# Picsart-AI-Research/MI-GAN

Hardware: AMD Instinct MI355X
Metric: images/sec migan-512 generator fwd (higher is better)
Workload: dtype f32; 1 GPU; migan-512 generator forward, batch=32 per GPU, 512x512, fp32 (BASELINE configs[2]); global_batch=32, resolution=512, parallelism=batch-shard x1, activation_storage=f32, streams=2, weights=static (migan_assume_static_weights: 1x1 operand planes prepared once)

## Files before the change

### mi-gan_amd/csrc/migan_pipe.hpp

```cpp
#pragma once

namespace migan {

constexpr int kPipeBWaves = 8;
constexpr int pipe_threads(int na) { return (na + kPipeBWaves) * 64; }

template <int MODE, int NT, int CIN, bool FROMRGB, int R>
struct PipeLds {
  static constexpr int NKC = CIN / 32;
  static constexpr int IN_SLOT = 1536 * 16;
  static constexpr int A_BUF = 2 * 128 * 64;
  static constexpr int B_CHUNK = 2 * NT * 64;
  static constexpr bool WRES = NKC * B_CHUNK <= 32 * 1024;
  static constexpr int NBUF_B = WRES ? NKC : 2;
  static constexpr int OFF_IN = 0;
  static constexpr int OFF_A = OFF_IN + R * IN_SLOT;
  static constexpr int OFF_B = OFF_A + 2 * A_BUF;
  static constexpr int OFF_W = OFF_B + NBUF_B * B_CHUNK;
  static constexpr bool TAPS_RES = NKC <= 8;
  static constexpr int OFF_F = OFF_W + (TAPS_RES ? NKC : 2) * 1280;
  static constexpr int F_SZ = FROMRGB ? NKC * 3 * 32 * 32 : 0;
  static constexpr int OFF_RGB = OFF_F + F_SZ;
  static constexpr int RGB_BUF = 192 * 32;
  static constexpr int OFF_T = OFF_RGB + (FROMRGB ? 2 * RGB_BUF : 0);
// ... 532 lines not shown

  if constexpr (MODE == MODE_NORMAL) {
    float* const t_s = reinterpret_cast<float*>(lds + L::OFF_T) + wb * (32 * 32);
    const int q4 = lane & 7, prow = lane >> 3;
    int twr[4];
    {
      const int u = (l31 >> 2) ^ (2 * half);
#pragma unroll
      for (int v = 0; v < 4; ++v) twr[v] = (4 * half) * 32 + ((u ^ ((v & 1) + 4 * (v >> 1))) << 2) + (l31 & 3);
    }
    const int trd0 = prow * 32 + ((q4 ^ (prow >> 1)) << 2), trd1 = prow * 32 + ((q4 ^ (prow >> 1) ^ 4) << 2);
    float nz[4] = {0.f, 0.f, 0.f, 0.f};
    float nzn[4] = {0.f, 0.f, 0.f, 0.f};
    float rs[4][3];
    unsigned pix0 = 0;
    f4 tw[NTIW][3];
    float tbias[3] = {0.f, 0.f, 0.f};
    if constexpr (TORGB) {
#pragma unroll
      for (int ch = 0; ch < 3; ++ch) tbias[ch] = p.trgb_b[ch];
#pragma unroll
      for (int j = 0; j < NTIW; ++j)
#pragma unroll
        for (int ch = 0; ch < 3; ++ch) tw[j][ch] = ld4(p.trgb_w + ch * p.CO + cbk * (NT / 2) + j * 32 + q4 * 4);
    }
    float* const part_s = reinterpret_cast<float*>(lds + L::OFF_P) + rb * (32 * 4);
    u4v u8c = {0u, 0u, 0u, 0u}, u8n = {0u, 0u, 0u, 0u};
    auto request_next = [&]() {
      if (has_noise) {
        const unsigned px = (unsigned)((cgy0 + 2 * rb) * p.WO + cgx0 + prow) * 4u;
#pragma unroll
        for (int q = 0; q < 4; ++q) nzn[q] = *at_bytes(p.noise + ((q >> 1) * p.WO + (q & 1) * 8), px);
      }
      if constexpr (TORGB) {
        if (p.u8_out && cbk == 0 && q4 < 4)
          u8n = fetch_pixel_bytes(p.u8_img, p.u8_mask, (size_t)cb0 * p.HO * p.WO + (size_t)(cgy0 + 2 * rb + (q4 >> 1)) * p.WO + cgx0 + (q4 & 1) * 8 + prow);
      }
    };
    auto begin_tile_epilogue = [&]() {
      pix0 = (unsigned)((pgy0 + 2 * rb) * p.WO + pgx0 + prow);
#pragma unroll
      for (int q = 0; q < 4; ++q) nz[q] = nzn[q];
      if constexpr (TORGB) {
        u8c = u8n;
#pragma unroll
        for (int q = 0; q < 4; ++q) rs[q][0] = rs[q][1] = rs[q][2] = 0.0f;
      }
    };
    auto stage_block = [&](const f16v& a) {
      MIGAN_WAVE_SYNC();
#pragma unroll
      for (int r = 0; r < 16; ++r) t_s[twr[((r >> 1) & 1) + 2 * ((r >> 2) & 1)] + ((r & 3) + 8 * (r >> 2)) * 32] = a[r];
      MIGAN_WAVE_SYNC();
    };
    f4 tv[4];
    auto fetch_block = [&]() {
#pragma unroll
      for (int q = 0; q < 4; ++q) tv[q] = ld4(t_s + ((q & 1) ? trd1 : trd0) + q * 8 * 32);
    };
    auto finish_block = [&](int j) {
      char* yb = reinterpret_cast<char*>(p.y) + (size_t)pb0 * img_out_bytes;
#pragma unroll
      for (int q = 0; q < 4; ++q) {
        f4 v = tv[q] * acc_scale + MIGAN_FMUL_RN(nz[q], ns);
        v = act4(v);
        const unsigned pix = pix0 + (unsigned)((q >> 1) * p.WO + (q & 1) * 8);
        Io<0>::st(yb, (pix * (unsigned)p.CO + (unsigned)(pn0 + cbk * (NT / 2) + j * 32 + q4 * 4)) * 4u, v);
        if constexpr (TORGB) {
          float r0, r1, r2;
          torgb_partial(v, tw[j][0], tw[j][1], tw[j][2], r0, r1, r2);
          rs[q][0] += r0; rs[q][1] += r1; rs[q][2] += r2;
        }
      }
    };
    float mine[3] = {0.f, 0.f, 0.f};
    auto rgb_partials = [&]() {
#pragma unroll
      for (int q = 0; q < 4; ++q) {
        const float s0 = MIGAN_SUM8(rs[q][0]), s1 = MIGAN_SUM8(rs[q][1]), s2 = MIGAN_SUM8(rs[q][2]);
        if (q4 == q) { mine[0] = s0; mine[1] = s1; mine[2] = s2; }
      }
      if (cbk == 1 && q4 < 4) st4(part_s + (8 * q4 + prow) * 4, f4{mine[0], mine[1], mine[2], 0.0f});
    };
    auto rgb_finish = [&]() {
      if (cbk == 0 && q4 < 4) {
        const f4 other = ld4(part_s + (8 * q4 + prow) * 4);
        const size_t plane = (size_t)p.HO * p.WO;
        const int oy = pgy0 + 2 * rb + (q4 >> 1), ox = pgx0 + (q4 & 1) * 8 + prow;
        float o3[3] = {mine[0] + other.x, mine[1] + other.y, mine[2] + other.z};
        MIGAN_OPAQUE_F(o3[0]); MIGAN_OPAQUE_F(o3[1]); MIGAN_OPAQUE_F(o3[2]);
        o3[0] += tbias[0]; MIGAN_OPAQUE_F(o3[0]);
        o3[1] += tbias[1]; MIGAN_OPAQUE_F(o3[1]);
        o3[2] += tbias[2]; MIGAN_OPAQUE_F(o3[2]);
        if (p.img_prev) {
          const int y0 = (oy & 1) ? (oy >> 1) : (oy >> 1) - 1, x0 = (ox & 1) ? (ox >> 1) : (ox >> 1) - 1;
          const float wy0 = (oy & 1) ? 0.75f : 0.25f, wx0 = (ox & 1) ? 0.75f : 0.25f;
          const float* pw = reinterpret_cast<const float*>(lds + L::OFF_PW + ppar * L::PW_SZ) + (y0 - (pgy0 >> 1) + 1) * 10 + (x0 - (pgx0 >> 1) + 1);
#pragma unroll
          for (int ch = 0; ch < 3; ++ch) {
            const float r0 = wx0 * pw[ch * 64] + (1.0f - wx0) * pw[ch * 64 + 1];
            const float r1 = wx0 * pw[ch * 64 + 10] + (1.0f - wx0) * pw[ch * 64 + 11];
            o3[ch] = (wy0 * r0 + (1.0f - wy0) * r1) + o3[ch];
          }
        }
        if (p.u8_out) {
          compose_pixel_bytes(u8c, p.u8_out, (size_t)pb0 * plane + (size_t)oy * p.WO + ox, o3[0], o3[1], o3[2]);
        } else {
          const unsigned po = (unsigned)(oy * p.WO + ox) * 4u;
#pragma unroll
          for (int ch = 0; ch < 3; ++ch) *at_bytes(p.img_out + ((size_t)pb0 * 3 + ch) * plane, po) = o3[ch];
        }
      }
    };
#pragma unroll
    for (int c = 0; c < NKC; ++c) {
      mfma_chunk(c & 1, WRES ? c : (c & 1), c == 0);
      if (c == NKC - 1) {
        request_next();
        stage_block(acc[0]);
        hand_over();
      }
      if constexpr (FROMRGB) build_step(bcur);
      MIGAN_BARRIER_LDS();
    }
    for (int t = 1; t < T; ++t) {
#pragma unroll
      for (int c = 0; c < NKC; ++c) {
        PPROF_MARK(7);
        if (c < NTIW) fetch_block();
        mfma_chunk(c & 1, WRES ? c : (c & 1), c == 0);
        PPROF_MARK(4);
        if (c == NKC - 1) request_next();
        PPROF_MARK(12);
        if (c == 0) begin_tile_epilogue();
        PPROF_MARK(5);
        if (c < NTIW) {
          finish_block(c);
          if (c + 1 < NTIW) stage_block(accp[c + 1 < NTIW ? c + 1 : 0]);
        }
        PPROF_MARK(9);
        if constexpr (TORGB) {
          if (c == NTIW - 1) rgb_partials();
          PPROF_MARK(10);
          if (c == NTIW) rgb_finish();
          PPROF_MARK(11);
        }
        if (c == NKC - 1) {
          stage_block(acc[0]);
          hand_over();
        }
        PPROF_MARK(7);
        if constexpr (FROMRGB) build_step(bcur);
        PPROF_MARK(13);
        MIGAN_BARRIER_LDS();
        PPROF_MARK(6);
      }
    }
    begin_tile_epilogue();
#pragma unroll
    for (int j = 0; j < NTIW; ++j) {
      fetch_block();
      finish_block(j);
      if (j + 1 < NTIW) stage_block(accp[j + 1 < NTIW ? j + 1 : 0]);
    }
    if constexpr (TORGB) {
      rgb_partials();
      MIGAN_BARRIER_LDS();
      rgb_finish();
    }
  } else {
    constexpr int GS = 64 + 4, QN = 16, LG_QN = 4, NH = NT / 64;
    static_assert(NT == 64 || NT == 128, "FIR-up tiles: 64 or 128 output channels");
    constexpr int SP = NKC / NH;
    static_assert(NKC % NH == 0 && SP >= 2, "too few K steps to hide the FIR epilogue under");
    constexpr int BT = kPipeBWaves * 64;
    constexpr int STEP = BT >> LG_QN;
    constexpr int ITEMS = MT * QN / BT;
    float* const g_s = reinterpret_cast<float*>(lds + L::OFF_T);
    auto acc_to_lds = [&](int h) {
      if (NH == 2 && cbk != h) return;
#pragma unroll
      for (int j = 0; j < NTIW; ++j)
#pragma unroll
        for (int r = 0; r < 16; ++r) {
          const int row = rb * 32 + (r & 3) + 8 * (r >> 2) + 4 * half;
          const int ly = pgy0 + (row >> lgGW), lx = pgx0 + (row & (GW - 1));
          float v = accp[j][r];
          if (ly < 0 || ly >= p.H || lx < 0 || lx >= p.W) v = 0.0f;
          g_s[row * GS + (NH == 2 ? j * 32 : cbk * 32) + l31] = v;
        }
    };
    const int c4 = tb & (QN - 1), m0 = tb >> LG_QN;
    struct ItemIo {
      f4 sk[2][2];
      float nzv[2][2];
    };
    auto item_geo = [&](int k, int h, int& m, unsigned& lpix, unsigned& loff) -> bool {
      m = m0 + k * STEP;
      const int gy = m >> lgGW, gx = m & (GW - 1);
      if (gy < 1 || gy > GH - 2 || gx < 1 || gx > GW - 2) return false;
      const int ly = pgy0 + gy, lx = pgx0 + gx;
      if (ly >= p.H || lx >= p.W) return false;
      lpix = (unsigned)((2 * ly) * p.WO + 2 * lx);
      loff = (lpix * (unsigned)p.CO + (unsigned)(pn0 + h * 64 + c4 * 4)) * 4u;
      return true;
    };
    auto item_load = [&](int k, int h, ItemIo& io) {
      int m;
      unsigned lpix, loff;
      if (!item_geo(k, h, m, lpix, loff)) return;
      const char* sb = p.skip ? reinterpret_cast<const char*>(p.skip) + (size_t)pb0 * img_out_bytes : nullptr;
#pragma unroll
      for (int a = 0; a < 2; ++a)
#pragma unroll
        for (int bb = 0; bb < 2; ++bb) {
          const unsigned dp = (unsigned)(a * p.WO + bb);
          io.nzv[a][bb] = has_noise ? p.noise[lpix + dp] : 0.0f;
          io.sk[a][bb] = sb ? Io<0>::ld_once(sb, loff + dp * (unsigned)p.CO * 4u) : f4{0.f, 0.f, 0.f, 0.f};
        }
    };
    auto item_finish = [&](int k, int h, const ItemIo& io) {
      int m;
      unsigned lpix, loff;
      if (!item_geo(k, h, m, lpix, loff)) return;
      char* yb = reinterpret_cast<char*>(p.y) + (size_t)pb0 * img_out_bytes;
      f4 e[3], o[3];
#pragma unroll
      for (int dy = 0; dy < 3; ++dy) {
        const float* gp = g_s + (m + (dy - 1) * GW) * GS + c4 * 4;
        const f4 l = ld4(gp - GS), ctr = ld4(gp), rgt = ld4(gp + GS);
        e[dy] = 0.25f * l + 0.75f * ctr;
        o[dy] = 0.75f * ctr + 0.25f * rgt;
      }
      f4 out[2][2];
      out[0][0] = 0.25f * e[0] + 0.75f * e[1];
      out[0][1] = 0.25f * o[0] + 0.75f * o[1];
      out[1][0] = 0.75f * e[1] + 0.25f * e[2];
      out[1][1] = 0.75f * o[1] + 0.25f * o[2];
#pragma unroll
      for (int a = 0; a < 2; ++a)
#pragma unroll
        for (int bb = 0; bb < 2; ++bb) {
          f4 v = out[a][bb] * acc_scale + MIGAN_FMUL_RN(io.nzv[a][bb], ns);
          v = act4(v);
          v += io.sk[a][bb];
          Io<0>::st(yb, loff + (unsigned)(a * p.WO + bb) * (unsigned)p.CO * 4u, v);
        }
    };
    constexpr int SL = SP - 1;
    auto slice_of = [](int k) { return k * SL / ITEMS; };
    ItemIo io[2];
#pragma unroll
    for (int c = 0; c < NKC; ++c) {
      mfma_chunk(c & 1, WRES ? c : (c & 1), c == 0);
      if (c == NKC - 1) hand_over();
      MIGAN_BARRIER_LDS();
    }
    for (int t = 1; t < T; ++t) {
#pragma unroll
      for (int c = 0; c < NKC; ++c) {
        constexpr int dummy = 0; (void)dummy;
        const int h = c / SP, cs = c % SP;
        if (cs >= 1) {
#pragma unroll
          for (int k = 0; k < ITEMS; ++k)
            if (slice_of(k) == cs - 1 && (k == 0 || slice_of(k - 1) != cs - 1)) item_load(k, h, io[k & 1]);
        }
        PPROF_MARK(7);
        mfma_chunk(c & 1, WRES ? c : (c & 1), c == 0);
        PPROF_MARK(4);
        if (cs == 0) {
          acc_to_lds(h);
        } else {
#pragma unroll
          for (int k = 0; k < ITEMS; ++k)
            if (slice_of(k) == cs - 1) {
              if (k + 1 < ITEMS && slice_of(k + 1) == cs - 1) item_load(k + 1, h, io[(k + 1) & 1]);
              item_finish(k, h, io[k & 1]);
            }
        }
        if (c == NKC - 1) hand_over();
        PPROF_MARK(5);
        MIGAN_BARRIER_LDS();
        PPROF_MARK(6);
      }
    }
#pragma unroll
    for (int h = 0; h < NH; ++h) {
      if (h > 0) MIGAN_BARRIER_LDS();
      acc_to_lds(h);
      MIGAN_BARRIER_LDS();
      item_load(0, h, io[0]);
#pragma unroll
      for (int k = 0; k < ITEMS; ++k) {
        if (k + 1 < ITEMS) item_load(k + 1, h, io[(k + 1) & 1]);
        item_finish(k, h, io[k & 1]);
      }
    }
  }
  PPROF_MARK(5);
  PPROF_END(AT);
}

template <int NT, int CIN, int R>
struct DownLds {
  static constexpr int KC = 16, NKC = CIN / KC;
  static constexpr int IN_UNITS = 12 * 36 * 4;
  static constexpr int A_BUF = 2 * 64 * 32;
  static constexpr int B_CHUNK = 2 * NT * 32;
  static constexpr bool WRES = NKC * B_CHUNK <= 32 * 1024;
  static constexpr int NBUF_B = WRES ? NKC : 2;
  static constexpr int DWP = 17;
  static constexpr int D_SZ = 10 * 2 * DWP * KC * 4;
  static constexpr int IN_SLOT = IN_UNITS * 16;
  static constexpr int OFF_D = R * IN_SLOT;
  static constexpr int OFF_A = OFF_D + D_SZ;
  static constexpr int OFF_B = OFF_A + 2 * A_BUF;
  static constexpr int OFF_W = OFF_B + NBUF_B * B_CHUNK;
  static constexpr int OFF_T = OFF_W + NKC * 640;
  template <int NB> static constexpr int total() { return OFF_T + NB * 32 * 32 * 4; }
};

template <int NT, int CIN, int R, int NA, int NB>
MIGAN_GLOBAL void MIGAN_LAUNCH_BOUNDS((NA + NB) * 64, (NA + NB) / 4) sepconv_pipedown_kernel(const SepArgs p) {
  typedef DownLds<NT, CIN, R> L;
  constexpr int AT = NA * 64, KC = 16, QC = 4, LG_QC = 2, NKC = L::NKC, MT = 64, GH = 4, GW = 16, lgGW = 4;
  constexpr int IGH = 12, IGW = 36, NPIXW = IGH * IGW, NITEMS = NPIXW * QC, DH = 10, DW = 34, DH2 = 5, DWP = L::DWP;
  constexpr int DNI = (NITEMS + AT - 1) / AT;
  constexpr bool WRES = L::WRES;
  constexpr int DNB = (4 * NT + AT - 1) / AT;
  static_assert(NB == 4 || NB == 8, "2 row blocks x 2 or 4 column groups");
  constexpr int NTIW = NT * 2 / (32 * NB);
  constexpr bool DEFER = NTIW <= 2;
  static_assert(NTIW <= NKC, "one epilogue block per K step");
  static_assert(NT == 128 || NT == 256, "one workgroup owns 128 or 256 output channels");
  static_assert(R == 2, "two-slot ring");
  static_assert(L::template total<NB>() <= 160 * 1024, "LDS budget");
  MIGAN_DYN_SMEM(smem);
  char* const lds = reinterpret_cast<char*>(smem);
  constexpr int IN_SLOT = L::IN_SLOT, OFF_D = L::OFF_D, OFF_A = L::OFF_A, OFF_B = L::OFF_B, OFF_W = L::OFF_W, OFF_T = L::OFF_T;

  const int tid = threadIdx.x;
  const int lane = tid & 63;
  const int wave_u = MIGAN_UNIFORM(tid >> 6);
  const bool groupA = tid < AT;
  const int HO = p.H >> 1, WO = p.W >> 1;

  const int ntiles = p.tiles_x * p.tiles_y * p.nchunks * p.B;
  const int xcd = (int)blockIdx.x & 7;
  const int tq = ntiles >> 3, tr = ntiles & 7;
  const int tcnt = tq + (xcd < tr ? 1 : 0);
  const int tbase = xcd < tr ? xcd * (tq + 1) : tr * (tq + 1) + (xcd - tr) * tq;
  const int tstep = ((int)gridDim.x + 7 - xcd) >> 3;
  const int tl0 = (int)blockIdx.x >> 3;
  const int T = tl0 < tcnt ? (tcnt - tl0 + tstep - 1) / tstep : 0;
  if (T == 0) return;
  const int G = T * NKC;
  PPROF_BEGIN();
  struct TileCur {
    int n, x, y, b;
  };
  const int st_n = tstep % p.nchunks, st_r1 = tstep / p.nchunks;
  const int st_x = st_r1 % p.tiles_x, st_r2 = st_r1 / p.tiles_x;
  const int st_y = st_r2 % p.tiles_y, st_b = st_r2 / p.tiles_y;
  TileCur tile0;
  {
    int t = tbase + tl0;
    tile0.n = t % p.nchunks; t /= p.nchunks;
    tile0.x = t % p.tiles_x; t /= p.tiles_x;
    tile0.y = t % p.tiles_y;
    tile0.b = t / p.tiles_y;
  }
  auto tile_next = [&](TileCur& c) {
    int carry = 0;
    c.n += st_n;
    if (c.n >= p.nchunks) { c.n -= p.nchunks; carry = 1; }
    c.x += st_x + carry; carry = 0;
    if (c.x >= p.tiles_x) { c.x -= p.tiles_x; carry = 1; }
    c.y += st_y + carry; carry = 0;
    if (c.y >= p.tiles_y) { c.y -= p.tiles_y; carry = 1; }
    c.b += st_b + carry;
  };

  if (groupA) {
    MIGAN_SETPRIO(2);
    const int lt = tid;
    float* const w_s = reinterpret_cast<float*>(lds + OFF_W);
    float* const d_s = reinterpret_cast<float*>(lds + OFF_D);
    for (int i = lt; i < CIN * 9 / 4; i += AT) {
      const f4 v = ld4(p.wdw + i * 4);
#pragma unroll
      for (int e = 0; e < 4; ++e) {
        const int f = i * 4 + e, ch = f / 9, tap = f - ch * 9;
        w_s[(ch >> 4) * 160 + tap * 16 + (ch & 15)] = v[e];
      }
    }
    for (int i = lt; i < CIN / 4; i += AT) st4(w_s + ((i * 4) >> 4) * 160 + 144 + ((i * 4) & 15), ld4(p.bdw + i * 4));

    const MIGAN_BUF wbuf = MIGAN_MAKE_BUF(p.wsplit, (unsigned)(2 * p.CO * CIN) * 2u);
    const bool bshort = MIGAN_UNIFORM((DNB - 1) * AT + wave_u * 64) >= 4 * NT;
    unsigned dboff[DNB];
#pragma unroll
    for (int j = 0; j < DNB; ++j) {
      const int u = lt + j * AT;
      const int plane = u / (2 * NT), rem = u % (2 * NT);
      dboff[j] = (unsigned)(plane * p.CO * CIN + (rem >> 1) * 32 + (rem & 1) * 8) * 2u;
    }
    auto dma_b = [&](int n0_, int chunk, int buf) {
      float* bb = reinterpret_cast<float*>(lds + OFF_B + buf * L::B_CHUNK);
      const unsigned soff = (unsigned)((chunk >> 1) * 32 * p.CO + n0_ * 32 + (chunk & 1) * 16) * 2u;
#pragma unroll
      for (int j = 0; j < DNB; ++j)
        if (j + 1 < DNB || !bshort) MIGAN_LDS_DMA16(wbuf, dboff[j], soff, bb + (j * AT + wave_u * 64) * 4);
    };
    const bool dshort = MIGAN_UNIFORM((DNI - 1) * AT + wave_u * 64) >= NITEMS;
    unsigned dgoff[DNI], drel[DNI], tile_soff = 0;
#pragma unroll
    for (int j = 0; j < DNI; ++j) {
      const int i = lt + j * AT;
      drel[j] = 0xfffff000u;
      if (i < NITEMS) {
        const int c4 = i & (QC - 1), pix = i >> LG_QC;
        drel[j] = (unsigned)(((pix / IGW) * p.W + (pix % IGW)) * CIN + c4 * 4) * 4u;
      }
    }
    auto make_dgoff = [&](int gy0_, int gx0_) {
      const int iy0 = 2 * gy0_ - 2, ix0 = 2 * gx0_ - 2;
      if (iy0 >= 0 && iy0 + IGH <= p.H && ix0 >= 0 && ix0 + IGW <= p.W) {
#pragma unroll
        for (int j = 0; j < DNI; ++j) dgoff[j] = drel[j];
        tile_soff = (unsigned)((iy0 * p.W + ix0) * CIN) * 4u;
        return;
      }
      tile_soff = 0;
#pragma unroll
      for (int j = 0; j < DNI; ++j) {
        const int i = lt + j * AT;
        unsigned g = 0xfffff000u;
        if (i < NITEMS) {
          const int c4 = i & (QC - 1), pix = i >> LG_QC;
          const int yy = iy0 + pix / IGW, xx = ix0 + pix % IGW;
          if (yy >= 0 && yy < p.H && xx >= 0 && xx < p.W) g = (unsigned)((yy * p.W + xx) * CIN + c4 * 4) * 4u;
        }
        dgoff[j] = g;
      }
    };
    const unsigned img_bytes = (unsigned)(p.H * p.W * CIN) * 4u;
    auto dma_in = [&](int b0_, int chunk, int slot) {
      float* in_s = reinterpret_cast<float*>(lds + slot * IN_SLOT);
      const MIGAN_BUF xbuf = MIGAN_MAKE_BUF(reinterpret_cast<const char*>(p.x) + (size_t)b0_ * img_bytes, img_bytes);
#pragma unroll
      for (int j = 0; j < DNI; ++j)
        if (j + 1 < DNI || !dshort) MIGAN_LDS_DMA16(xbuf, dgoff[j], tile_soff + (unsigned)(chunk * KC) * 4u, in_s + (j * AT + wave_u * 64) * 4);
    };
    auto stage1 = [&](int slot, int chunk, int gy0_, int gx0_) {
      const float* in_s = reinterpret_cast<const float*>(lds + slot * IN_SLOT);
      const float* wc = w_s + chunk * 160;
      const int c4 = lt & (QC - 1);
      f4 w[9];
#pragma unroll
      for (int tap = 0; tap < 9; ++tap) w[tap] = ld4(wc + tap * KC + c4 * 4);
      const f4 bias = ld4(wc + KC * 9 + c4 * 4);
      const int yim0 = 2 * gy0_ - 1, xim0 = 2 * gx0_ - 1;
      for (int it = lt; it < DH2 * DW * QC; it += AT) {
        const int r = it >> LG_QC;
        const int dx = r % DW, dy0 = 2 * (r / DW);
        const float* ip = in_s + (dy0 * IGW + dx) * KC + c4 * 4;
        f4 win[4][3];
#pragma unroll
        for (int rr = 0; rr < 4; ++rr) {
          win[rr][0] = ld4(ip); win[rr][1] = ld4(ip + KC); win[rr][2] = ld4(ip + 2 * KC);
          ip += IGW * KC;
        }
        const int xim = xim0 + dx;
        const bool colin = xim >= 0 && xim < p.W;
        float* dp = d_s + ((dy0 * 2 + (dx & 1)) * DWP + (dx >> 1)) * KC + c4 * 4;
        f4 dv[2];
#pragma unroll
        for (int o = 0; o < 2; ++o) {
          f4 sacc = bias;
#pragma unroll
          for (int ky = 0; ky < 3; ++ky)
#pragma unroll
            for (int kx = 0; kx < 3; ++kx) sacc += w[ky * 3 + kx] * win[o + ky][kx];
          const int yim = yim0 + dy0 + o;
          dv[o] = f4{0.f, 0.f, 0.f, 0.f};
          if (colin && yim >= 0 && yim < p.H) dv[o] = act4(sacc);
        }
        st4(dp, 0.125f * dv[0] + 0.375f * dv[1]);
        st4(dp + 2 * DWP * KC, 0.375f * dv[0] + 0.125f * dv[1]);
      }
    };
    auto stage2 = [&](int abuf) {
      char* a_b = lds + OFF_A + abuf * L::A_BUF;
      for (int it = lt; it < MT * QC; it += AT) {
        const int c4 = it & (QC - 1), m = it >> LG_QC;
        const int ox = m & (GW - 1), oy = m >> lgGW;
        const float* dp = d_s + ((2 * oy) * 2 * DWP + ox) * KC + c4 * 4;
        f4 a = {0.f, 0.f, 0.f, 0.f};
#pragma unroll
        for (int kx = 0; kx < 4; ++kx) {
          const float fx = (kx == 0 || kx == 3) ? 0.125f : 0.375f;
          const float* q = dp + ((kx & 1) * DWP + (kx >> 1)) * KC;
          a += fx * (ld4(q) + ld4(q + 3 * 2 * DWP * KC));
        }
        u2v h1, h2;
        split2_f16(a * kF16AScale, h1, h2);
        char* d = a_b + m * 32 + c4 * 8;
        *reinterpret_cast<u2v*>(d) = h1;
        *reinterpret_cast<u2v*>(d + MT * 32) = h2;
      }
    };

    int is = 0, ic = 0, ik = 0, ib0 = 0, in0 = 0, igy0 = 0, igx0 = 0;
    TileCur itc = tile0;
    auto icoords = [&]() { in0 = itc.n * NT; ib0 = itc.b; igy0 = itc.y * GH; igx0 = itc.x * GW; };
    icoords();
    make_dgoff(igy0, igx0);
    auto issue = [&]() {
      if (is < G) {
        dma_in(ib0, ic, is & 1);
        ++is;
        if (++ic == NKC) {
          ic = 0;
          if (++ik < T) { tile_next(itc); icoords(); make_dgoff(igy0, igx0); }
        }
      }
    };
    int bs = 0, bc = 0, bk = 0, bn0 = in0;
    TileCur btc = tile0;
    auto issue_b = [&]() -> bool {
      if (bs >= G) return false;
      dma_b(bn0, bc, bs & 1);
      ++bs;
      if (++bc == NKC) {
        bc = 0;
        if (++bk < T) { tile_next(btc); bn0 = btc.n * NT; }
      }
      return true;
    };
    int dk = 0, dc = 0, dgy0 = igy0, dgx0 = igx0;
    TileCur dtc = tile0;
    auto dadvance = [&]() {
      if (++dc == NKC) {
        dc = 0;
        if (++dk < T) { tile_next(dtc); dgy0 = dtc.y * GH; dgx0 = dtc.x * GW; }
      }
    };
    if constexpr (WRES) {
#pragma unroll
      for (int c = 0; c < NKC; ++c) dma_b(in0, c, c);
    } else {
      issue_b();
      issue_b();
    }
    issue();
    issue();
    if (dshort) MIGAN_WAIT_VMCNT(DNI - 1); else MIGAN_WAIT_VMCNT(DNI);
    MIGAN_BARRIER_LDS();
    stage1(0, 0, dgy0, dgx0);
    MIGAN_BARRIER_LDS();
    stage2(0);
    dadvance();
    MIGAN_WAIT_VMCNT(0);
    MIGAN_BARRIER_LDS();
    for (int g = 0; g < G; ++g) {
      issue();
      PPROF_MARK(0);
      if (g + 1 < G) stage1((g + 1) & 1, dc, dgy0, dgx0);
      PPROF_MARK(1);
      MIGAN_BARRIER_LDS();
      PPROF_MARK(3);
      if (g + 1 < G) { stage2((g + 1) & 1); dadvance(); }
      PPROF_MARK(14);
      bool newer = false;
      if constexpr (!WRES) newer = issue_b();
      if (newer && !bshort) MIGAN_WAIT_VMCNT(DNB); else if (newer && DNB > 1) MIGAN_WAIT_VMCNT(DNB > 1 ? DNB - 1 : 0); else MIGAN_WAIT_VMCNT(0);
      PPROF_MARK(2);
      MIGAN_BARRIER_LDS();
      PPROF_MARK(3);
    }
    PPROF_END(AT);
    return;
  }

  const int wb = wave_u - NA;
  const int rb = wb & 1, cb = wb >> 1;
  const int l31 = lane & 31, half = lane >> 5;
  f16v acc[NTIW], accp[DEFER ? NTIW : 1];
#pragma unroll
  for (int j = 0; j < NTIW; ++j)
#pragma unroll
    for (int r = 0; r < 16; ++r) { acc[j][r] = 0.0f; if (DEFER) accp[j][r] = 0.0f; }
  auto mfma_chunk = [&](int abuf, int bbuf, bool first) {
    const char* ab = lds + OFF_A + abuf * L::A_BUF + (rb * 32 + l31) * 32 + half * 16;
    const char* bb = lds + OFF_B + bbuf * L::B_CHUNK + half * 16;
    const f4 a_hi = ld4(reinterpret_cast<const float*>(ab)), a_lo = ld4(reinterpret_cast<const float*>(ab + MT * 32));
    f4 b_hi[NTIW], b_lo[NTIW];
#pragma unroll
    for (int j = 0; j < NTIW; ++j) {
      const char* q = bb + ((cb * NTIW + j) * 32 + l31) * 32;
      b_hi[j] = ld4(reinterpret_cast<const float*>(q));
      b_lo[j] = ld4(reinterpret_cast<const float*>(q + NT * 32));
      if (first) acc[j] = f16v{0.f, 0.f, 0.f, 0.f, 0.f, 0.f, 0.f, 0.f, 0.f, 0.f, 0.f, 0.f, 0.f, 0.f, 0.f, 0.f};
    }
#pragma unroll
    for (int j = 0; j < NTIW; ++j) acc[j] = MIGAN_MFMA_F16_32X32X16(a_lo, b_hi[j], acc[j]);
#pragma unroll
    for (int j = 0; j < NTIW; ++j) acc[j] = MIGAN_MFMA_F16_32X32X16(a_hi, b_lo[j], acc[j]);
#pragma unroll
    for (int j = 0; j < NTIW; ++j) acc[j] = MIGAN_MFMA_F16_32X32X16(a_hi, b_hi[j], acc[j]);
  };
  const float acc_scale = reinterpret_cast<const float*>(p.wsplit)[-4];
  const float gain_s = 1.41421356237309515f * acc_scale;
  const size_t img_out_bytes = (size_t)HO * WO * p.CO * 4;
  int ck = 0, cn0 = 0, cb0 = 0, cgy0 = 0, cgx0 = 0, pn0 = 0, pb0 = 0, pgy0 = 0, pgx0 = 0;
  TileCur ctc = tile0;
  auto ccoords = [&]() { cn0 = ctc.n * NT; cb0 = ctc.b; cgy0 = ctc.y * GH; cgx0 = ctc.x * GW; };
  ccoords();
  float* const t_s = reinterpret_cast<float*>(lds + OFF_T) + wb * (32 * 32);
  const int q4 = lane & 7, prow = lane >> 3;
  int twr[4];
  {
    const int u = (l31 >> 2) ^ (2 * half);
#pragma unroll
    for (int v = 0; v < 4; ++v) twr[v] = (4 * half) * 32 + ((u ^ ((v & 1) + 4 * (v >> 1))) << 2) + (l31 & 3);
  }
  const int trd0 = prow * 32 + ((q4 ^ (prow >> 1)) << 2), trd1 = prow * 32 + ((q4 ^ (prow >> 1) ^ 4) << 2);
  auto stage_block = [&](const f16v& a) {
    MIGAN_WAVE_SYNC();
#pragma unroll
    for (int r = 0; r < 16; ++r) t_s[twr[((r >> 1) & 1) + 2 * ((r >> 2) & 1)] + ((r & 3) + 8 * (r >> 2)) * 32] = a[r];
    MIGAN_WAVE_SYNC();
  };
  f4 tv[4];
  auto fetch_block = [&]() {
#pragma unroll
    for (int q = 0; q < 4; ++q) tv[q] = ld4(t_s + ((q & 1) ? trd1 : trd0) + q * 8 * 32);
  };
  auto finish_block = [&](int j) {
    char* yb = reinterpret_cast<char*>(p.y) + (size_t)pb0 * img_out_bytes;
    const unsigned pix0 = (unsigned)((pgy0 + 2 * rb) * WO + pgx0 + prow);
#pragma unroll
    for (int q = 0; q < 4; ++q) {
      const f4 v = act4g(tv[q], gain_s);
      const unsigned pix = pix0 + (unsigned)((q >> 1) * WO + (q & 1) * 8);
      Io<0>::st(yb, (pix * (unsigned)p.CO + (unsigned)(pn0 + (cb * NTIW + j) * 32 + q4 * 4)) * 4u, v);
    }
  };
  auto hand_over = [&]() {
    pn0 = cn0; pb0 = cb0; pgy0 = cgy0; pgx0 = cgx0;
    if constexpr (DEFER) {
      stage_block(acc[0]);
#pragma unroll
      for (int j = 1; j < NTIW; ++j) accp[j] = acc[j];
    } else {
#pragma unroll
      for (int j = 0; j < NTIW; ++j) {
        stage_block(acc[j]);
        fetch_block();
        finish_block(j);
      }
    }
    if (++ck < T) { tile_next(ctc); ccoords(); }
  };
  MIGAN_BARRIER_LDS();
  MIGAN_BARRIER_LDS();
  MIGAN_BARRIER_LDS();
  if constexpr (!DEFER) {
    for (int t = 0; t < T; ++t) {
#pragma unroll
      for (int c = 0; c < NKC; ++c) {
        PPROF_MARK(7);
        mfma_chunk(c & 1, WRES ? c : (c & 1), c == 0);
        PPROF_MARK(4);
        MIGAN_BARRIER_LDS();
        PPROF_MARK(6);
        if (c == NKC - 1) hand_over();
        PPROF_MARK(9);
        MIGAN_BARRIER_LDS();
        PPROF_MARK(6);
      }
    }
    PPROF_END(AT);
    return;
  } else {
#pragma unroll
  for (int c = 0; c < NKC; ++c) {
    mfma_chunk(c & 1, WRES ? c : (c & 1), c == 0);
    MIGAN_BARRIER_LDS();
    if (c == NKC - 1) hand_over();
    MIGAN_BARRIER_LDS();
  }
  for (int t = 1; t < T; ++t) {
#pragma unroll
    for (int c = 0; c < NKC; ++c) {
      PPROF_MARK(7);
      mfma_chunk(c & 1, WRES ? c : (c & 1), c == 0);
      PPROF_MARK(4);
      MIGAN_BARRIER_LDS();
      PPROF_MARK(6);
      if (c < NTIW) {
        fetch_block();
        finish_block(c);
        if (c + 1 < NTIW) stage_block(accp[c + 1 < NTIW ? c + 1 : 0]);
      }
      PPROF_MARK(9);
      if (c == NKC - 1) hand_over();
      PPROF_MARK(7);
      MIGAN_BARRIER_LDS();
      PPROF_MARK(6);
    }
  }
#pragma unroll
  for (int j = 0; j < NTIW; ++j) {
    fetch_block();
    finish_block(j);
    if (j + 1 < NTIW) stage_block(accp[j + 1 < NTIW ? j + 1 : 0]);
  }
  PPROF_MARK(9);
  PPROF_END(AT);
  }
}

}
```

### mi-gan_amd/csrc/migan_pipe_table.inc

```
namespace migan {
#define MIGAN_P(MODE, NT, CIN, RGB, TORGB, R, NA)                                                                                \
  {MODE, NT, CIN, RGB, TORGB, R, NA, sepconv_pipe_kernel<MODE, NT, CIN, RGB, TORGB, R, NA>,                                      \
   "migan::sepconv_pipe_kernel<" #MODE ", " #NT ", " #CIN ", " #RGB ", " #TORGB ", " #R ", " #NA ">", (size_t)PipeLds<MODE, NT, CIN, RGB, R>::TOTAL}
PipeSlice pipe_slice() {
  static const PipeEntry t[] = {
      MIGAN_P(0, 64, 64, false, false, 3, 4), MIGAN_P(0, 64, 64, false, true, 3, 4), MIGAN_P(0, 64, 64, true, false, 2, 4),
      MIGAN_P(0, 64, 64, false, false, 3, 8), MIGAN_P(0, 64, 64, false, true, 3, 8), MIGAN_P(0, 64, 64, true, false, 2, 8),
      MIGAN_P(0, 128, 128, false, false, 2, 4), MIGAN_P(0, 128, 128, false, true, 2, 4),
      MIGAN_P(2, 64, 128, false, false, 2, 4),
  };
  return PipeSlice{t, (int)(sizeof(t) / sizeof(t[0]))};
}
#undef MIGAN_P
#define MIGAN_D(NT, CIN, R, NA, NB)                                                                                              \
  {NT, CIN, R, NA, NB, sepconv_pipedown_kernel<NT, CIN, R, NA, NB>,                                                              \
   "migan::sepconv_pipedown_kernel<" #NT ", " #CIN ", " #R ", " #NA ", " #NB ">", (size_t)DownLds<NT, CIN, R>::template total<NB>()}
DownSlice pipedown_slice() {
  static const DownEntry t[] = {
      MIGAN_D(128, 64, 2, 4, 8), MIGAN_D(128, 64, 2, 8, 8), MIGAN_D(128, 64, 2, 12, 4),
      MIGAN_D(256, 128, 2, 4, 8), MIGAN_D(256, 128, 2, 12, 4),
  };
  return DownSlice{t, (int)(sizeof(t) / sizeof(t[0]))};
}
#undef MIGAN_D
}
```

Baseline: 3549 images/sec.

## Double-buffer depthwise scratch to overlap stage1 and stage2 in pipedown kernel

```diff
diff --git a/mi-gan_amd/csrc/migan_pipe.hpp b/mi-gan_amd/csrc/migan_pipe.hpp
--- a/mi-gan_amd/csrc/migan_pipe.hpp
+++ b/mi-gan_amd/csrc/migan_pipe.hpp
@@ -858,7 +858,7 @@
   PPROF_END(AT);
 }
 
-template <int NT, int CIN, int R>
+template <int NT, int CIN, int R, int NB = 4>
 struct DownLds {
   static constexpr int KC = 16, NKC = CIN / KC;
   static constexpr int IN_UNITS = 12 * 36 * 4;
@@ -869,17 +869,20 @@
   static constexpr int DWP = 17;
   static constexpr int D_SZ = 10 * 2 * DWP * KC * 4;
   static constexpr int IN_SLOT = IN_UNITS * 16;
+  static constexpr int T_SZ = NB * 32 * 32 * 4;
+  static constexpr int REST = R * IN_SLOT + 2 * A_BUF + NBUF_B * B_CHUNK + NKC * 640 + T_SZ;
+  static constexpr bool OVL = REST + 2 * D_SZ <= 160 * 1024;
   static constexpr int OFF_D = R * IN_SLOT;
-  static constexpr int OFF_A = OFF_D + D_SZ;
+  static constexpr int OFF_A = OFF_D + (OVL ? 2 : 1) * D_SZ;
   static constexpr int OFF_B = OFF_A + 2 * A_BUF;
   static constexpr int OFF_W = OFF_B + NBUF_B * B_CHUNK;
   static constexpr int OFF_T = OFF_W + NKC * 640;
-  template <int NB> static constexpr int total() { return OFF_T + NB * 32 * 32 * 4; }
+  static constexpr int TOTAL = OFF_T + T_SZ;
 };
 
 template <int NT, int CIN, int R, int NA, int NB>
 MIGAN_GLOBAL void MIGAN_LAUNCH_BOUNDS((NA + NB) * 64, (NA + NB) / 4) sepconv_pipedown_kernel(const SepArgs p) {
-  typedef DownLds<NT, CIN, R> L;
+  typedef DownLds<NT, CIN, R, NB> L;
   constexpr int AT = NA * 64, KC = 16, QC = 4, LG_QC = 2, NKC = L::NKC, MT = 64, GH = 4, GW = 16, lgGW = 4;
   constexpr int IGH = 12, IGW = 36, NPIXW = IGH * IGW, NITEMS = NPIXW * QC, DH = 10, DW = 34, DH2 = 5, DWP = L::DWP;
   constexpr int DNI = (NITEMS + AT - 1) / AT;
@@ -891,7 +894,8 @@
   static_assert(NTIW <= NKC, "one epilogue block per K step");
   static_assert(NT == 128 || NT == 256, "one workgroup owns 128 or 256 output channels");
   static_assert(R == 2, "two-slot ring");
-  static_assert(L::template total<NB>() <= 160 * 1024, "LDS budget");
+  static_assert(L::TOTAL <= 160 * 1024, "LDS budget");
+  constexpr bool OVL = L::OVL;
   MIGAN_DYN_SMEM(smem);
   char* const lds = reinterpret_cast<char*>(smem);
   constexpr int IN_SLOT = L::IN_SLOT, OFF_D = L::OFF_D, OFF_A = L::OFF_A, OFF_B = L::OFF_B, OFF_W = L::OFF_W, OFF_T = L::OFF_T;
@@ -1009,63 +1013,109 @@
       for (int j = 0; j < DNI; ++j)
         if (j + 1 < DNI || !dshort) MIGAN_LDS_DMA16(xbuf, dgoff[j], tile_soff + (unsigned)(chunk * KC) * 4u, in_s + (j * AT + wave_u * 64) * 4);
     };
-    auto stage1 = [&](int slot, int chunk, int gy0_, int gx0_) {
+    constexpr int N1 = DH2 * DW * QC, NP1 = (N1 + AT - 1) / AT;
+    constexpr int DBUF = L::D_SZ / 4;
+    const int c4 = lt & (QC - 1);
+    f4 win[4][3], w[9], bias;
+    auto s1_on = [&](int k) -> bool { return MIGAN_UNIFORM(k * AT + wave_u * 64) < N1; };
+    auto s1_taps = [&](int chunk) __attribute__((always_inline)) {
+      const float* wc = w_s + chunk * 160;
+#pragma unroll
+      for (int tap = 0; tap < 9; ++tap) w[tap] = ld4(wc + tap * KC + c4 * 4);
+      bias = ld4(wc + KC * 9 + c4 * 4);
+    };
+    auto s1_load = [&](int k, int slot) __attribute__((always_inline)) {
       const float* in_s = reinterpret_cast<const float*>(lds + slot * IN_SLOT);
-      const float* wc = w_s + chunk * 160;
-      const int c4 = lt & (QC - 1);
-      f4 w[9];
-#pragma unroll
-      for (int tap = 0; tap < 9; ++tap) w[tap] = ld4(wc + tap * KC + c4 * 4);
-      const f4 bias = ld4(wc + KC * 9 + c4 * 4);
-      const int yim0 = 2 * gy0_ - 1, xim0 = 2 * gx0_ - 1;
-      for (int it = lt; it < DH2 * DW * QC; it += AT) {
-        const int r = it >> LG_QC;
-        const int dx = r % DW, dy0 = 2 * (r / DW);
-        const float* ip = in_s + (dy0 * IGW + dx) * KC + c4 * 4;
-        f4 win[4][3];
-#pragma unroll
-        for (int rr = 0; rr < 4; ++rr) {
-          win[rr][0] = ld4(ip); win[rr][1] = ld4(ip + KC); win[rr][2] = ld4(ip + 2 * KC);
-          ip += IGW * KC;
-        }
-        const int xim = xim0 + dx;
-        const bool colin = xim >= 0 && xim < p.W;
-        float* dp = d_s + ((dy0 * 2 + (dx & 1)) * DWP + (dx >> 1)) * KC + c4 * 4;
-        f4 dv[2];
-#pragma unroll
-        for (int o = 0; o < 2; ++o) {
-          f4 sacc = bias;
-#pragma unroll
-          for (int ky = 0; ky < 3; ++ky)
-#pragma unroll
-            for (int kx = 0; kx < 3; ++kx) sacc += w[ky * 3 + kx] * win[o + ky][kx];
-          const int yim = yim0 + dy0 + o;
-          dv[o] = f4{0.f, 0.f, 0.f, 0.f};
-          if (colin && yim >= 0 && yim < p.H) dv[o] = act4(sacc);
-        }
+      const int it = lt + k * AT < N1 ? lt + k * AT : c4;
+      const int r = it >> LG_QC;
+      const int dx = r % DW, dy0 = 2 * (r / DW);
+      const float* ip = in_s + (dy0 * IGW + dx) * KC + c4 * 4;
+#pragma unroll
+      for (int rr = 0; rr < 4; ++rr) {
+        win[rr][0] = ld4(ip); win[rr][1] = ld4(ip + KC); win[rr][2] = ld4(ip + 2 * KC);
+        ip += IGW * KC;
+      }
+    };
+    auto s1_finish = [&](int k, int dbuf, int gy0_, int gx0_) __attribute__((always_inline)) {
+      const bool mine = lt + k * AT < N1;
+      const int it = mine ? lt + k * AT : c4;
+      const int r = it >> LG_QC;
+      const int dx = r % DW, dy0 = 2 * (r / DW);
+      const int yim0 = 2 * gy0_ - 1, xim = 2 * gx0_ - 1 + dx;
+      const bool colin = xim >= 0 && xim < p.W;
+      float* dp = d_s + dbuf * DBUF + ((dy0 * 2 + (dx & 1)) * DWP + (dx >> 1)) * KC + c4 * 4;
+      f4 dv[2];
+#pragma unroll
+      for (int o = 0; o < 2; ++o) {
+        f4 sacc = bias;
+#pragma unroll
+        for (int ky = 0; ky < 3; ++ky)
+#pragma unroll
+          for (int kx = 0; kx < 3; ++kx) sacc += w[ky * 3 + kx] * win[o + ky][kx];
+        const int yim = yim0 + dy0 + o;
+        dv[o] = f4{0.f, 0.f, 0.f, 0.f};
+        if (colin && yim >= 0 && yim < p.H) dv[o] = act4(sacc);
+      }
+      if (mine) {
         st4(dp, 0.125f * dv[0] + 0.375f * dv[1]);
         st4(dp + 2 * DWP * KC, 0.375f * dv[0] + 0.125f * dv[1]);
       }
     };
-    auto stage2 = [&](int abuf) {
-      char* a_b = lds + OFF_A + abuf * L::A_BUF;
-      for (int it = lt; it < MT * QC; it += AT) {
-        const int c4 = it & (QC - 1), m = it >> LG_QC;
-        const int ox = m & (GW - 1), oy = m >> lgGW;
-        const float* dp = d_s + ((2 * oy) * 2 * DWP + ox) * KC + c4 * 4;
-        f4 a = {0.f, 0.f, 0.f, 0.f};
-#pragma unroll
-        for (int kx = 0; kx < 4; ++kx) {
-          const float fx = (kx == 0 || kx == 3) ? 0.125f : 0.375f;
-          const float* q = dp + ((kx & 1) * DWP + (kx >> 1)) * KC;
-          a += fx * (ld4(q) + ld4(q + 3 * 2 * DWP * KC));
-        }
-        u2v h1, h2;
-        split2_f16(a * kF16AScale, h1, h2);
-        char* d = a_b + m * 32 + c4 * 8;
-        *reinterpret_cast<u2v*>(d) = h1;
-        *reinterpret_cast<u2v*>(d + MT * 32) = h2;
-      }
+    constexpr int N2 = MT * 8, S2OFF = AT > N2 ? AT - N2 : 0, NP2 = N2 / (AT - S2OFF);
+    static_assert((AT - S2OFF) * NP2 == N2 && NP2 <= NP1 && S2OFF % 64 == 0, "stage-2 items tile the upper threads of group A");
+    const bool s2_on = wave_u * 64 >= S2OFF;
+    f2v fa[4], fb[4];
+    auto s2_load = [&](int k, int dbuf) __attribute__((always_inline)) {
+      const int it = lt - S2OFF + k * (AT - S2OFF);
+      const int c2 = it & 7, m = it >> 3;
+      const int ox = m & (GW - 1), oy = m >> lgGW;
+      const float* dp = d_s + dbuf * DBUF + ((2 * oy) * 2 * DWP + ox) * KC + c2 * 2;
+#pragma unroll
+      for (int kx = 0; kx < 4; ++kx) {
+        const float* q = dp + ((kx & 1) * DWP + (kx >> 1)) * KC;
+        fa[kx] = *reinterpret_cast<const f2v*>(q);
+        fb[kx] = *reinterpret_cast<const f2v*>(q + 3 * 2 * DWP * KC);
+      }
+    };
+    auto s2_finish = [&](int k, int abuf) __attribute__((always_inline)) {
+      const int it = lt - S2OFF + k * (AT - S2OFF);
+      const int c2 = it & 7, m = it >> 3;
+      f2v a = {0.f, 0.f};
+#pragma unroll
+      for (int kx = 0; kx < 4; ++kx) {
+        const float fx = (kx == 0 || kx == 3) ? 0.125f : 0.375f;
+        a += fx * (fa[kx] + fb[kx]);
+      }
+      const f2v v = a * kF16AScale;
+      const unsigned h1 = MIGAN_PACK_F16(v.x, v.y);
+      const unsigned h2 = MIGAN_PACK_F16(v.x - MIGAN_F16LO_F32(h1), v.y - MIGAN_F16HI_F32(h1));
+      char* d = lds + OFF_A + abuf * L::A_BUF + m * 32 + c2 * 4;
+      *reinterpret_cast<unsigned*>(d) = h1;
+      *reinterpret_cast<unsigned*>(d + MT * 32) = h2;
+    };
+    auto part = [&](auto do2, auto do1, int ab, int db2, int slot, int db1, int chunk, int gy0_, int gx0_) __attribute__((always_inline)) {
+      constexpr bool D2 = decltype(do2)::value, D1 = decltype(do1)::value;
+      if (D2) s2_load(0, db2);
+#pragma unroll
+      for (int k = 0; k < NP1; ++k) {
+        const bool on1 = D1 && (NP1 == 1 || k * AT + (NA - 1) * 64 < N1 || s1_on(k));
+        if (on1) s1_load(k, slot);
+        if (D1 && D2) MIGAN_SCHED_FENCE();
+        if (D2 && k < NP2) {
+          s2_finish(k, ab);
+          if (k + 1 < NP2) s2_load(k + 1, db2);
+        }
+        if (D1 && D2) MIGAN_SCHED_FENCE();
+        if (D1 && k == 0) s1_taps(chunk);
+        if (on1) s1_finish(k, db1, gy0_, gx0_);
+      }
+    };
+    auto interval = [&](auto do2, auto do1, int ab, int db2, int slot, int db1, int chunk, int gy0_, int gx0_) __attribute__((always_inline)) {
+      constexpr bool D2 = decltype(do2)::value, D1 = decltype(do1)::value;
+      const bool w2 = D2 && s2_on, w1 = D1 && (NP1 > 1 || s1_on(0));
+      if (w2 && w1) part(TrueT{}, TrueT{}, ab, db2, slot, db1, chunk, gy0_, gx0_);
+      else if (w1) part(FalseT{}, TrueT{}, ab, db2, slot, db1, chunk, gy0_, gx0_);
+      else if (w2) part(TrueT{}, FalseT{}, ab, db2, slot, db1, chunk, gy0_, gx0_);
     };
 
     int is = 0, ic = 0, ik = 0, ib0 = 0, in0 = 0, igy0 = 0, igx0 = 0;
@@ -1106,7 +1156,7 @@
     if constexpr (WRES) {
 #pragma unroll
       for (int c = 0; c < NKC; ++c) dma_b(in0, c, c);
-    } else {
+    } else if constexpr (!OVL) {
       issue_b();
       issue_b();
     }
@@ -1114,27 +1164,51 @@
     issue();
     if (dshort) MIGAN_WAIT_VMCNT(DNI - 1); else MIGAN_WAIT_VMCNT(DNI);
     MIGAN_BARRIER_LDS();
-    stage1(0, 0, dgy0, dgx0);
-    MIGAN_BARRIER_LDS();
-    stage2(0);
+    interval(FalseT{}, TrueT{}, 0, 0, 0, 0, dc, dgy0, dgx0);
     dadvance();
-    MIGAN_WAIT_VMCNT(0);
-    MIGAN_BARRIER_LDS();
-    for (int g = 0; g < G; ++g) {
-      issue();
-      PPROF_MARK(0);
-      if (g + 1 < G) stage1((g + 1) & 1, dc, dgy0, dgx0);
-      PPROF_MARK(1);
-      MIGAN_BARRIER_LDS();
-      PPROF_MARK(3);
-      if (g + 1 < G) { stage2((g + 1) & 1); dadvance(); }
-      PPROF_MARK(14);
-      bool newer = false;
-      if constexpr (!WRES) newer = issue_b();
-      if (newer && !bshort) MIGAN_WAIT_VMCNT(DNB); else if (newer && DNB > 1) MIGAN_WAIT_VMCNT(DNB > 1 ? DNB - 1 : 0); else MIGAN_WAIT_VMCNT(0);
-      PPROF_MARK(2);
-      MIGAN_BARRIER_LDS();
-      PPROF_MARK(3);
+    if constexpr (OVL) {
+      MIGAN_WAIT_VMCNT(0);
+      MIGAN_BARRIER_LDS();
+      int q = 0;
+      for (int g = -1; g < G - 2; ++g) {
+        issue();
+        if constexpr (!WRES) issue_b();
+        PPROF_MARK(0);
+        interval(TrueT{}, TrueT{}, q, q, q ^ 1, q ^ 1, dc, dgy0, dgx0);
+        dadvance();
+        PPROF_MARK(1);
+        MIGAN_WAIT_VMCNT(0);
+        PPROF_MARK(2);
+        MIGAN_BARRIER_LDS();
+        PPROF_MARK(3);
+        q ^= 1;
+      }
+      if constexpr (!WRES) issue_b();
+      interval(TrueT{}, FalseT{}, q, q, 0, 0, 0, 0, 0);
+      MIGAN_WAIT_VMCNT(0);
+      MIGAN_BARRIER_LDS();
+      MIGAN_BARRIER_LDS();
+    } else {
+      MIGAN_BARRIER_LDS();
+      interval(TrueT{}, FalseT{}, 0, 0, 0, 0, 0, 0, 0);
+      MIGAN_WAIT_VMCNT(0);
+      MIGAN_BARRIER_LDS();
+      for (int g = 0; g < G; ++g) {
+        issue();
+        PPROF_MARK(0);
+        if (g + 1 < G) { interval(FalseT{}, TrueT{}, 0, 0, (g + 1) & 1, 0, dc, dgy0, dgx0); dadvance(); }
+        PPROF_MARK(1);
+        MIGAN_BARRIER_LDS();
+        PPROF_MARK(3);
+        if (g + 1 < G) interval(TrueT{}, FalseT{}, (g + 1) & 1, 0, 0, 0, 0, 0, 0);
+        PPROF_MARK(14);
+        bool newer = false;
+        if constexpr (!WRES) newer = issue_b();
+        if (newer && !bshort) MIGAN_WAIT_VMCNT(DNB); else if (newer && DNB > 1) MIGAN_WAIT_VMCNT(DNB > 1 ? DNB - 1 : 0); else MIGAN_WAIT_VMCNT(0);
+        PPROF_MARK(2);
+        MIGAN_BARRIER_LDS();
+        PPROF_MARK(3);
+      }
     }
     PPROF_END(AT);
     return;
@@ -1230,8 +1304,7 @@
         PPROF_MARK(7);
         mfma_chunk(c & 1, WRES ? c : (c & 1), c == 0);
         PPROF_MARK(4);
-        MIGAN_BARRIER_LDS();
-        PPROF_MARK(6);
+        if constexpr (!OVL) MIGAN_BARRIER_LDS();
         if (c == NKC - 1) hand_over();
         PPROF_MARK(9);
         MIGAN_BARRIER_LDS();
@@ -1244,7 +1317,7 @@
 #pragma unroll
   for (int c = 0; c < NKC; ++c) {
     mfma_chunk(c & 1, WRES ? c : (c & 1), c == 0);
-    MIGAN_BARRIER_LDS();
+    if constexpr (!OVL) MIGAN_BARRIER_LDS();
     if (c == NKC - 1) hand_over();
     MIGAN_BARRIER_LDS();
   }
@@ -1252,12 +1325,15 @@
 #pragma unroll
     for (int c = 0; c < NKC; ++c) {
       PPROF_MARK(7);
+      if (OVL && c < NTIW) fetch_block();
       mfma_chunk(c & 1, WRES ? c : (c & 1), c == 0);
       PPROF_MARK(4);
-      MIGAN_BARRIER_LDS();
-      PPROF_MARK(6);
+      if constexpr (!OVL) {
+        MIGAN_BARRIER_LDS();
+        PPROF_MARK(6);
+        if (c < NTIW) fetch_block();
+      }
       if (c < NTIW) {
-        fetch_block();
         finish_block(c);
         if (c + 1 < NTIW) stage_block(accp[c + 1 < NTIW ? c + 1 : 0]);
       }
diff --git a/mi-gan_amd/csrc/migan_pipe_table.inc b/mi-gan_amd/csrc/migan_pipe_table.inc
--- a/mi-gan_amd/csrc/migan_pipe_table.inc
+++ b/mi-gan_amd/csrc/migan_pipe_table.inc
@@ -14,7 +14,7 @@
 #undef MIGAN_P
 #define MIGAN_D(NT, CIN, R, NA, NB)                                                                                              \
   {NT, CIN, R, NA, NB, sepconv_pipedown_kernel<NT, CIN, R, NA, NB>,                                                              \
-   "migan::sepconv_pipedown_kernel<" #NT ", " #CIN ", " #R ", " #NA ", " #NB ">", (size_t)DownLds<NT, CIN, R>::template total<NB>()}
+   "migan::sepconv_pipedown_kernel<" #NT ", " #CIN ", " #R ", " #NA ", " #NB ">", (size_t)DownLds<NT, CIN, R, NB>::TOTAL}
 DownSlice pipedown_slice() {
   static const DownEntry t[] = {
       MIGAN_D(128, 64, 2, 4, 8), MIGAN_D(128, 64, 2, 8, 8), MIGAN_D(128, 64, 2, 12, 4),
```

Result: no change. 3548 images/sec, median of 3 (-0.0%).
